# ethz-asl/object_keypoints

Measured on AMD Instinct MI355X. Metric: frames/sec keypoint inference (511x511 -> heatmaps+3D), higher is better.
Workload: dtype bf16; 1 GPU; BASELINE configs[2]: batch=64/GPU synthetic 511x511 frames, bf16 activations+weights, fp32 accumulate, CornerNet-Squeeze K=3 (valve) random-init procedural weights; fp32 NCHW frames -> stem -> hourglass+heads; peak-NMS -> depth lifting -> object grouping on injected bump scenes (SURVEY 8(d), 1-2 objects/frame); frames_per_gpu=64, global_batch=64, parallelism=frame-dp1, resident_frame_batches=4

## Files before the change

### object_keypoints_amd/csrc/okp_igemm_patch.hip

```cpp
#include <cstdio>
#include <cstdlib>
#include <cstring>
#include <type_traits>
#include <vector>

#include "okp_igemm_kernel.h"


namespace {

constexpr uint32_t kPatchKeys = 0x7ac788u;
template <int MT> __device__ __forceinline__ uint32_t patch_key(int col) {
  return MT == 16 ? (kPatchKeys >> (3 * (col >> 1))) & 7u : (uint32_t)(col >> 1) & 7u;
}

constexpr int kWStage = 256 * 128;
constexpr int kPitch = 18;
constexpr int kPatchBuf = 41 * 1024;
constexpr int kLdsPatch = 2 * kWStage;
constexpr int kLdsSteps = kLdsPatch + 2 * kPatchBuf;
constexpr int kLdsBias = kLdsSteps + 256 * (int)sizeof(OkpPatchStep);
#ifdef OKP_PATCH_STAMPS
constexpr int kStampBytes = 1024;
__device__ __forceinline__ uint64_t stamp() { uint64_t t; asm volatile("s_memtime %0" : "=s"(t)); return t; }
#else
constexpr int kStampBytes = 0;
#endif
constexpr int kGeoEntries = 328;
constexpr int kLdsGeo = kLdsBias + 1024;
constexpr int kLdsStamps = kLdsGeo + OKP_PATCH_MAX_GEOM * kGeoEntries * 4;
constexpr int kLdsTotal = kLdsStamps + kStampBytes;
static_assert(sizeof(OkpPatchStep) == 16, "step table entries are read as one 16-byte vector");
static_assert(256 * 512 <= kLdsSteps, "epilogue staging (256 px x 256 ch bf16) must not reach the step table");
static_assert(kLdsTotal <= 160 * 1024, "one workgroup's LDS is at most the CU's 160 KiB");

template <typename T, int MT = 16, bool RG = false>
__global__ __launch_bounds__(512) void okp_igemm_patch_kernel(const OkpPatchParams p) {
  static_assert(!RG || std::is_same<T, _Float16>::value, "the 16-bit storage guard is an fp16 instantiation");
  using x4_t = typename H16<T>::x4;
  using x8_t = typename H16<T>::x8;
  static_assert(MT == 16 || MT == 32, "MFMA tile");
  constexpr int TCO = 64 / MT, TPX = 128 / MT;
  constexpr int AREGS = MT * MT / 64;
  using acc_t = typename Mma<T, MT>::acc_t;
  __shared__ __attribute__((aligned(16))) char smem[kLdsTotal];
  char* const steps_lds = smem + kLdsSteps;
  char* const bias_lds = smem + kLdsBias;

  const int tid = threadIdx.x;
  const int lane = tid & 63;
  const int wave = __builtin_amdgcn_readfirstlane(tid >> 6);
  const int wco = wave >> 1, wpx = wave & 1;
  const int fr = lane & 15, fh = lane >> 4;

  const __amdgpu_buffer_rsrc_t rs_w = __builtin_amdgcn_make_buffer_rsrc(const_cast<void*>(p.weights), 0, (int)p.w_bytes, 0x00020000);
  const __amdgpu_buffer_rsrc_t rs_b = __builtin_amdgcn_make_buffer_rsrc(const_cast<float*>(p.bias), 0, p.n_co_tiles * 256 * 4, 0x00020000);
  const __amdgpu_buffer_rsrc_t rs_s0 = __builtin_amdgcn_make_buffer_rsrc(const_cast<void*>(p.src_data[0]), 0, (int)p.src_bytes[0], 0x00020000);
  const __amdgpu_buffer_rsrc_t rs_s1 = __builtin_amdgcn_make_buffer_rsrc(const_cast<void*>(p.src_data[1]), 0, (int)p.src_bytes[1], 0x00020000);

  if (tid < p.n_steps) reinterpret_cast<u32x4*>(steps_lds)[tid] = reinterpret_cast<const u32x4*>(p.steps)[tid];
  __syncthreads();

  const int r0 = tid >> 3;
  const int wc = (tid & 7) ^ ((r0 >> 1) & 7);

  for (int slot = blockIdx.x; slot < p.n_tiles; slot += gridDim.x) {
    const int xq = p.n_tiles >> 3, xr = p.n_tiles & 7, xcd = slot & 7;
    const int tile = (xcd < xr ? xcd * (xq + 1) : xr * (xq + 1) + (xcd - xr) * xq) + (slot >> 3);
    const int cls = p.n_classes == 4 ? (tile & 3) : 0;
    const int tile_c = p.n_classes == 4 ? (tile >> 2) : tile;
    const int t0 = cls * p.steps_per_class, t1 = t0 + p.steps_per_class;
    const int co_tile = tile_c % p.n_co_tiles;
    const int px_tile = tile_c / p.n_co_tiles;
    const int n = fastdiv(px_tile, p.div_tiles_frame);
    const int trem = px_tile - n * p.tiles_y * p.tiles_x;
    const int tyi = fastdiv(trem, p.div_tiles_x);
    const int y0 = tyi * 16, x0 = (trem - tyi * p.tiles_x) * 16;
    const int co0 = co_tile * 256;

    if (wave == 0)
      __builtin_amdgcn_raw_ptr_buffer_load_lds(rs_b, (lds_ptr_t)bias_lds, 16, (int)((uint32_t)(co0 + lane * 4) * 4u), 0, 0, 0);

    uint32_t wbase[4];
#pragma unroll
    for (int i = 0; i < 4; ++i) {
      const int co = co0 + r0 + i * 64;
      wbase[i] = (co < p.cout_pad) ? (uint32_t)co * 128u + (uint32_t)wc * 16u : kInvalidOff;
    }

    auto issue_w = [&](int t, int stage) {
      const uint32_t wslice = (uint32_t)t * (uint32_t)p.cout_pad * 128u;
      char* const wt = smem + stage * kWStage + wave * 1024;
#pragma unroll
      for (int i = 0; i < 4; ++i)
        __builtin_amdgcn_raw_ptr_buffer_load_lds(rs_w, (lds_ptr_t)(wt + i * 8192), 16, (int)(wbase[i] + wslice), 0, 0, 0);
    };
    auto patch_pixel = [&](const OkpPatchGeom& G, int idx) -> uint32_t {
      const int i = idx / kPitch, j = idx - i * kPitch;
      const int ys = G.conv_stride * y0 + G.oy + i * G.step, xs = G.conv_stride * x0 + G.ox + j * G.step;
      const bool ok = idx < G.npx && j < G.PW && ys >= 0 && ys < G.H && xs >= 0 && xs < G.W;
      return ok ? ((uint32_t)((n * G.H + ys) * G.W + xs) * (uint32_t)(G.pix_stride * 2)) | patch_key<MT>(j) : kInvalidOff;
    };
    auto issue_patch_tab = [&](int geom, uint32_t c0b, int k0, int k1, int buf) {
      const int npx = 18 * (int)((p.geom_ph >> (5 * geom)) & 31u);
      const __amdgpu_buffer_rsrc_t rs_x = ((p.geom_src >> geom) & 1) ? rs_s1 : rs_s0;
      const uint32_t* const tab = reinterpret_cast<const uint32_t*>(smem + kLdsGeo) + geom * kGeoEntries + (lane >> 3);
      for (int k = k0; k < k1; ++k) {
        const int blk = k * 8 + wave;
        if (blk * 8 >= npx) continue;
        const uint32_t e = tab[blk * 8];
        const uint32_t off = (e & kInvalidOff) ? kInvalidOff : (e & ~7u) + c0b + ((((uint32_t)lane & 7u) ^ (e & 7u)) << 4);
        __builtin_amdgcn_raw_ptr_buffer_load_lds(rs_x, (lds_ptr_t)(smem + kLdsPatch + buf * kPatchBuf + blk * 1024), 16, (int)off, 0, 0, 0);
      }
    };
    auto issue_patch = [&](int geom, uint32_t c0b, int k0, int k1, int buf) {
      const OkpPatchGeom& G = p.g[geom];
      const int PW = G.PW, npx = G.npx;
      const int H = G.H, W = G.W, ps2 = G.pix_stride * 2, step = G.step;
      const int yb = G.conv_stride * y0 + G.oy, xb = G.conv_stride * x0 + G.ox;
      const __amdgpu_buffer_rsrc_t rs_x = __builtin_amdgcn_make_buffer_rsrc(const_cast<void*>(G.data), 0, (int)G.bytes, 0x00020000);
      for (int k = k0; k < k1; ++k) {
        const int blk = k * 8 + wave;
        if (blk * 8 >= npx) continue;
        const int idx = blk * 8 + (lane >> 3);
        const int i = idx / kPitch, j = idx - i * kPitch;
        const int ch = (lane & 7) ^ (int)patch_key<MT>(j);
        const int ys = yb + i * step, xs = xb + j * step;
        const bool ok = idx < npx && j < PW && ys >= 0 && ys < H && xs >= 0 && xs < W;
        const uint32_t off = ok ? (uint32_t)((n * H + ys) * W + xs) * (uint32_t)ps2 + c0b + (uint32_t)ch * 16u : kInvalidOff;
        char* const dst = smem + kLdsPatch + buf * kPatchBuf + blk * 1024;
        __builtin_amdgcn_raw_ptr_buffer_load_lds(rs_x, (lds_ptr_t)dst, 16, (int)off, 0, 0, 0);
      }
    };

    acc_t acc[TCO][TPX];
#pragma unroll
    for (int i = 0; i < TCO; ++i)
#pragma unroll
      for (int j = 0; j < TPX; ++j)
#pragma unroll
        for (int e = 0; e < AREGS; ++e) acc[i][j][e] = 0.f;

    for (int g = 0; g < p.n_geom; ++g)
      if (tid < kGeoEntries) reinterpret_cast<uint32_t*>(smem + kLdsGeo)[g * kGeoEntries + tid] = patch_pixel(p.g[g], tid);
    {
      const u32x4 s0 = *reinterpret_cast<const u32x4*>(steps_lds + t0 * 16);
      const uint32_t w3 = (uint32_t)__builtin_amdgcn_readfirstlane((int)s0[3]);
      const int g0 = w3 & 0xff;
      issue_patch(g0, ((w3 >> 16) & 0xffu) * 128u, 0, (p.g[g0].npx + 63) >> 6, __builtin_amdgcn_readfirstlane((int)s0[2]) & 0xff);
    }
    issue_w(t0, t0 & 1);

    for (int t = t0; t < t1; ++t) {
      const u32x4 sv = *reinterpret_cast<const u32x4*>(steps_lds + t * 16);
      const uint32_t tap_bytes = (uint32_t)__builtin_amdgcn_readfirstlane((int)sv[0]);
      const uint32_t nx_c0b = (uint32_t)__builtin_amdgcn_readfirstlane((int)sv[1]);
      const uint32_t pk = (uint32_t)__builtin_amdgcn_readfirstlane((int)sv[2]);
      const int pbuf = pk & 0xff, nx_k0 = (pk >> 8) & 0xff, nx_k1 = (pk >> 16) & 0xff, nx_geom = pk >> 24;
      const uint32_t w3 = (uint32_t)__builtin_amdgcn_readfirstlane((int)sv[3]);
      const int dxo = (w3 >> 8) & 0xff;
      const bool more = t + 1 < t1;
#ifdef OKP_PATCH_ABL_NOPATCH
      const bool next_patch = false; (void)nx_k0; (void)nx_k1; (void)nx_geom; (void)nx_c0b;
#else
      const bool next_patch = nx_k1 > nx_k0 && (int)(w3 >> 24) + 1 < t1;
#endif

#ifdef OKP_PATCH_STAMPS
      uint64_t T0 = stamp();
      asm volatile("s_waitcnt vmcnt(0) lgkmcnt(0)" ::: "memory");
      uint64_t T1 = stamp();
      asm volatile("s_waitcnt lgkmcnt(0)" ::: "memory");
      __builtin_amdgcn_s_barrier();
      uint64_t T2 = stamp();
#else
      asm volatile("s_waitcnt vmcnt(0) lgkmcnt(0)" ::: "memory");
      __builtin_amdgcn_s_barrier();
#endif

      const char* const wt = smem + (t & 1) * kWStage;
      const char* const pbase = smem + kLdsPatch + pbuf * kPatchBuf;
      if constexpr (MT == 32) {
        const int r32 = lane & 31, h32 = lane >> 5;
        const char* const bb = pbase + tap_bytes + (uint32_t)(((wpx * 8 + (r32 >> 4)) * kPitch + (r32 & 15)) * 128);
        const uint32_t bsw = patch_key<32>((r32 & 15) + dxo);
        auto lda = [&](int sub, int i) { return *reinterpret_cast<const u32x4*>(wt + swz<128>((wco * TCO + i) * 32 + r32, 2 * sub + h32)); };
        auto ldb = [&](int sub, int j) { return *reinterpret_cast<const u32x4*>(bb + j * (2 * kPitch * 128) + ((((uint32_t)(2 * sub + h32)) ^ bsw) << 4)); };
        u32x4 fa[2][TCO], fb[2][TPX];
#pragma unroll
        for (int i = 0; i < TCO; ++i) fa[0][i] = lda(0, i);
#pragma unroll
        for (int j = 0; j < TPX; ++j) fb[0][j] = ldb(0, j);
        if (more) issue_w(t + 1, (t + 1) & 1);
#pragma unroll
        for (int sub = 0; sub < 4; ++sub) {
          __builtin_amdgcn_sched_barrier(0);
          if (sub + 1 < 4) {
#pragma unroll
            for (int i = 0; i < TCO; ++i) fa[(sub + 1) & 1][i] = lda(sub + 1, i);
#pragma unroll
            for (int j = 0; j < TPX; ++j) fb[(sub + 1) & 1][j] = ldb(sub + 1, j);
          }
          if (sub == 1 && next_patch) issue_patch_tab(nx_geom, nx_c0b, nx_k0, nx_k1, pbuf ^ 1);
          __builtin_amdgcn_sched_barrier(0);
#pragma unroll
          for (int i = 0; i < TCO; ++i)
#pragma unroll
            for (int j = 0; j < TPX; ++j) acc[i][j] = H16<T>::mfma32(fa[sub & 1][i], fb[sub & 1][j], acc[i][j]);
        }
      } else {
      const char* const bb = pbase + tap_bytes + (uint32_t)((wpx * TPX * kPitch + fr) * 128);
      const uint32_t bsw = patch_key<16>(fr + dxo);
      auto lda = [&](int kk, int i) {
        return *reinterpret_cast<const u32x4*>(wt + swz<128>((wco * TCO + i) * 16 + fr, 4 * kk + fh));
      };
      auto ldb = [&](int kk, int j) {
        return *reinterpret_cast<const u32x4*>(bb + j * (kPitch * 128) + ((((uint32_t)(4 * kk + fh)) ^ bsw) << 4));
      };
      auto mma8 = [&](const u32x4 (&a)[TCO], const u32x4 (&bq)[2], auto s) {
        constexpr int S = decltype(s)::value;
#pragma unroll
        for (int i = 0; i < TCO; ++i)
#pragma unroll
          for (int h = 0; h < 2; ++h)
            acc[i][2 * S + h] = H16<T>::mfma16(a[i], bq[h], acc[i][2 * S + h]);
      };
      using S0 = std::integral_constant<int, 0>; using S1 = std::integral_constant<int, 1>;
      using S2 = std::integral_constant<int, 2>; using S3 = std::integral_constant<int, 3>;
      u32x4 a0[TCO], a1[TCO], bq0[2], bq1[2];
#pragma unroll
      for (int i = 0; i < TCO; ++i) a0[i] = lda(0, i);
      bq0[0] = ldb(0, 0); bq0[1] = ldb(0, 1);
      bq1[0] = ldb(0, 2); bq1[1] = ldb(0, 3);
      if (more) issue_w(t + 1, (t + 1) & 1);
      __builtin_amdgcn_sched_barrier(0);
      mma8(a0, bq0, S0{});
      __builtin_amdgcn_sched_barrier(0);
#ifdef OKP_PATCH_STAMPS
      {
        uint64_t T3 = stamp();
        asm volatile("s_waitcnt lgkmcnt(0)" : "+s"(T0), "+s"(T1), "+s"(T2), "+s"(T3) :: "memory");
        if (slot == (int)blockIdx.x && lane == 0 && t - t0 < kStampBytes / 128)
          *reinterpret_cast<u32x4*>(smem + kLdsStamps + ((t - t0) * 8 + wave) * 16) = u32x4{(uint32_t)T0, (uint32_t)T1, (uint32_t)T2, (uint32_t)T3};
      }
      __builtin_amdgcn_sched_barrier(0);
#endif
      bq0[0] = ldb(0, 4); bq0[1] = ldb(0, 5); a1[0] = lda(1, 0); a1[1] = lda(1, 1);
      __builtin_amdgcn_sched_barrier(0);
      mma8(a0, bq1, S1{});
      __builtin_amdgcn_sched_barrier(0);
      bq1[0] = ldb(0, 6); bq1[1] = ldb(0, 7); a1[2] = lda(1, 2); a1[3] = lda(1, 3);
      __builtin_amdgcn_sched_barrier(0);
      mma8(a0, bq0, S2{});
      __builtin_amdgcn_sched_barrier(0);
      bq0[0] = ldb(1, 0); bq0[1] = ldb(1, 1);
      if (next_patch) issue_patch_tab(nx_geom, nx_c0b, nx_k0, nx_k1, pbuf ^ 1);
      __builtin_amdgcn_sched_barrier(0);
      mma8(a0, bq1, S3{});
      __builtin_amdgcn_sched_barrier(0);
      bq1[0] = ldb(1, 2); bq1[1] = ldb(1, 3);
      __builtin_amdgcn_sched_barrier(0);
      mma8(a1, bq0, S0{});
      __builtin_amdgcn_sched_barrier(0);
      bq0[0] = ldb(1, 4); bq0[1] = ldb(1, 5);
      __builtin_amdgcn_sched_barrier(0);
      mma8(a1, bq1, S1{});
      __builtin_amdgcn_sched_barrier(0);
      bq1[0] = ldb(1, 6); bq1[1] = ldb(1, 7);
      __builtin_amdgcn_sched_barrier(0);
      mma8(a1, bq0, S2{});
      mma8(a1, bq1, S3{});
          }
    }
#ifdef OKP_PATCH_STAMPS
    {
      uint64_t TE = stamp();
      asm volatile("s_waitcnt lgkmcnt(0)" : "+s"(TE) :: "memory");
      if (slot == (int)blockIdx.x && lane == 0 && t1 - t0 < kStampBytes / 128)
        *reinterpret_cast<u32x4*>(smem + kLdsStamps + ((t1 - t0) * 8 + wave) * 16) = u32x4{(uint32_t)TE, 0u, 0u, 0u};
    }
    __syncthreads();
    if (slot == (int)blockIdx.x && blockIdx.x < 16 && p.dbg)
      for (int i = tid; i < kStampBytes / 4; i += 512) p.dbg[blockIdx.x * (kStampBytes / 4) + i] = reinterpret_cast<const uint32_t*>(smem + kLdsStamps)[i];
#endif
    __syncthreads();

#pragma unroll
    for (int i = 0; i < TCO; ++i) {
#pragma unroll
      for (int g = 0; g < AREGS / 4; ++g) {
        const int co_l = (wco * TCO + i) * MT + (MT == 32 ? 8 * g + 4 * (lane >> 5) : 4 * fh);
        const f32x4 bv = *reinterpret_cast<const f32x4*>(bias_lds + co_l * 4);
#pragma unroll
        for (int j = 0; j < TPX; ++j) {
          const int prow = (wpx * TPX + j) * MT + (lane & (MT - 1));
          char* dst = smem + prow * 512 + ((((co_l * 2) >> 4) ^ (prow & 7)) << 4) + ((co_l * 2) & 15);
          x4_t o;
#pragma unroll
          for (int e = 0; e < 4; ++e) o[e] = (T)(acc[i][j][4 * g + e] + bv[e]);
          *reinterpret_cast<x4_t*>(dst) = o;
        }
      }
    }
    __syncthreads();
    constexpr int U = 256 * 32 / 512;
    constexpr int UH = 8;
    const bool relu = p.act == OKP_ACT_RELU;
    uint32_t range_h = 0u;
#pragma unroll 1
    for (int ub = 0; ub < U; ub += UH) {
      u32x4 rres[UH];
      uint32_t ooff[UH];
#pragma unroll
      for (int u = 0; u < UH; ++u) {
        const int it = tid + (ub + u) * 512;
        const int q = it & 31, prow = it >> 5;
        const int co = co0 + q * 8;
        const uint32_t opix = (uint32_t)((n * p.OH + (y0 + (prow >> 4)) * p.out_step + p.out_oy + (cls >> 1)) * p.OW + (x0 + (prow & 15)) * p.out_step + p.out_ox + (cls & 1));
        ooff[u] = co < p.cout ? opix : kInvalidOff;
      }
      if (p.res) {
#pragma unroll
        for (int u = 0; u < UH; ++u) {
          const int q = (tid + (ub + u) * 512) & 31;
          const int co = co0 + q * 8;
          const uint32_t opix = ooff[u] == kInvalidOff ? 0u : ooff[u];
          rres[u] = *reinterpret_cast<const u32x4*>(static_cast<const char*>(p.res) + ((size_t)opix * p.res_pix_stride + (co < p.cout ? co : 0)) * 2);
        }
      }
#pragma unroll
      for (int u = 0; u < UH; ++u) {
        const int it = tid + (ub + u) * 512;
        const int q = it & 31, prow = it >> 5;
        u32x4 w = *reinterpret_cast<const u32x4*>(smem + prow * 512 + ((q ^ (prow & 7)) << 4));
        if (ooff[u] == kInvalidOff) continue;
        char* op = static_cast<char*>(p.out) + ((size_t)ooff[u] * p.out_pix_stride + co0 + q * 8) * 2;
        if (!p.res) {
          if (relu) {
            typedef short s16x8 __attribute__((ext_vector_type(8)));
            const s16x8 z = {0, 0, 0, 0, 0, 0, 0, 0};
            w = __builtin_bit_cast(u32x4, __builtin_elementwise_max(__builtin_bit_cast(s16x8, w), z));
          }
          if constexpr (RG) range_h = okp_range_max_h8(range_h, w);
          *reinterpret_cast<u32x4*>(op) = w;
        } else {
          const x8_t s8 = __builtin_bit_cast(x8_t, w), r8 = __builtin_bit_cast(x8_t, rres[u]);
          x8_t o;
#pragma unroll
          for (int e = 0; e < 8; ++e) {
            float v = (float)s8[e] + (float)r8[e];
            if (relu) v = fmaxf(v, 0.f);
            o[e] = (T)v;
          }
          if constexpr (RG) range_h = okp_range_max_h8(range_h, __builtin_bit_cast(u32x4, o));
          *reinterpret_cast<x8_t*>(op) = o;
        }
      }
    }
    if constexpr (RG) okp_raise_range_flag(p.range_flag, okp_range_exceeded_h2(range_h));
    __syncthreads();
  }
}

}

bool okp_patch_supported(const okp_conv* plan, const OkpIgemmParams& p) {
  const bool x3 = plan->dtype == OKP_F32X3;
  if (!plan->patch_steps_dev || !(okp_is16(plan->dtype) || x3)) return false;
  if ((p.n_classes != 1 && p.n_classes != 4) || p.dw_w) return false;
  if (p.Ho % 16 || p.Wo % 16) return false;
  if (x3 && (p.out16 || p.res16 || p.out_sub2 || !p.out || plan->n_single_slices)) return false;
  for (int s = 0; s < plan->n_src; ++s) {
    if (p.src_pix_stride[s] < plan->cin[s]) return false;
    if ((p.src_pix_stride[s] * okp_esz(plan->dtype)) % 8) return false;
  }
  return true;
}

int okp_fill_patch_params(const okp_conv* plan, const OkpIgemmParams& q, OkpPatchParams& p) {
  std::memset(&p, 0, sizeof(p));
  for (int gi = 0; gi < plan->patch_n_geom; ++gi) {
    const int ss = plan->patch_src[gi];
    OkpPatchGeom& g = p.g[gi];
// ... 16 lines not shown
  p.weights = q.weights; p.w_bytes = q.w_bytes; p.cout_pad = q.cout_pad; p.cout = q.cout; p.bias = q.bias; p.oscale = q.oscale;
  p.steps = plan->patch_steps_dev; p.n_steps = plan->n_slices;
  p.n_classes = q.n_classes; p.steps_per_class = plan->n_slices / q.n_classes;
  p.OH = q.OH; p.OW = q.OW; p.out_step = q.out_step; p.out_oy = q.out_oy; p.out_ox = q.out_ox;
  p.N = q.N; p.H = q.Ho; p.W = q.Wo; p.tiles_y = q.Ho / 16; p.tiles_x = q.Wo / 16;
  p.div_tiles_frame = okp_fastdiv((uint32_t)(p.tiles_y * p.tiles_x)); p.div_tiles_x = okp_fastdiv((uint32_t)p.tiles_x);
  p.out = q.out; p.out_bytes = q.out_bytes; p.out_pix_stride = q.out_pix_stride;
  p.res = q.res; p.res_bytes = q.res_bytes; p.res_pix_stride = q.res_pix_stride; p.act = q.act;
  p.pairs = ((uint32_t)q.src_pairs & 3u) | (q.out_pairs ? 4u : 0u);
  p.range_flag = q.range_flag;
  p.n_co_tiles = q.cout_pad / 256;
  p.tiles_per_class = p.n_co_tiles * p.N * p.tiles_y * p.tiles_x;
  p.n_tiles = p.tiles_per_class * p.n_classes;
  return OKP_OK;
}

int okp_launch_igemm_patch(const okp_conv* plan, const OkpIgemmParams& q, hipStream_t stream) {
  if (!okp_patch_supported(plan, q)) { okp_set_error("okp_conv_forward: tile 13 (patch-resident kernel) does not apply to this plan / problem"); return OKP_EINVAL; }
  OkpPatchParams p;
  if (int e = okp_fill_patch_params(plan, q, p)) return e;
  if (plan->dtype == OKP_F32X3) return okp_launch_igemm_patch_x3(plan, p, stream);
#ifdef OKP_PATCH_STAMPS
  static uint32_t* dbg = nullptr;
  if (!dbg) (void)hipMalloc((void**)&dbg, 16 * kStampBytes);
  (void)hipMemsetAsync(dbg, 0, 16 * kStampBytes, stream);
  p.dbg = dbg;
#endif
  const dim3 grid((unsigned)(p.n_tiles < 256 ? p.n_tiles : 256)), block(512);
  if (q.mfma32) {
    if (plan->dtype == OKP_BF16) hipLaunchKernelGGL((okp_igemm_patch_kernel<__bf16, 32>), grid, block, 0, stream, p);
    else if (p.range_flag) hipLaunchKernelGGL((okp_igemm_patch_kernel<_Float16, 32, true>), grid, block, 0, stream, p);
    else hipLaunchKernelGGL((okp_igemm_patch_kernel<_Float16, 32>), grid, block, 0, stream, p);
  } else if (plan->dtype == OKP_BF16) hipLaunchKernelGGL((okp_igemm_patch_kernel<__bf16, 16>), grid, block, 0, stream, p);
  else if (p.range_flag) hipLaunchKernelGGL((okp_igemm_patch_kernel<_Float16, 16, true>), grid, block, 0, stream, p);
  else hipLaunchKernelGGL((okp_igemm_patch_kernel<_Float16, 16>), grid, block, 0, stream, p);
#ifdef OKP_PATCH_STAMPS
  if (getenv("OKP_PATCH_STAMPS_PRINT")) {
    (void)hipStreamSynchronize(stream);
    std::vector<uint32_t> h(16 * kStampBytes / 4);
    (void)hipMemcpy(h.data(), dbg, 16 * kStampBytes, hipMemcpyDeviceToHost);
    const int ns = std::min(p.steps_per_class, kStampBytes / 128 - 1);
    printf("patch stamps: %d K-steps per tile; clocks per step: wait for the LDS-DMA | barrier | until the first MFMA group was issued | rest of the body\n", p.steps_per_class);
    for (int wg = 0; wg < 16; wg += 5)
      for (int t = 0; t < ns; ++t) {
        printf("wg %2d step %2d:", wg, t);
        for (int w = 0; w < 8; w += 7) {
          const uint32_t* a = &h[(size_t)wg * (kStampBytes / 4) + (t * 8 + w) * 4];
          printf("   wave %d: %5u | %5u | %5u | %5u", w, a[1] - a[0], a[2] - a[1], a[3] - a[2], a[32] - a[3]);
        }
        printf("\n");
      }
    double sum[4] = {0, 0, 0, 0};
    int cnt = 0;
    for (int wg = 0; wg < 16; ++wg)
      for (int t = 1; t < ns; ++t)
        for (int w = 0; w < 8; ++w) {
          const uint32_t* a = &h[(size_t)wg * (kStampBytes / 4) + (t * 8 + w) * 4];
          sum[0] += a[1] - a[0]; sum[1] += a[2] - a[1]; sum[2] += a[3] - a[2]; sum[3] += a[32] - a[3]; ++cnt;
        }
    printf("mean over 16 workgroups, all waves, steps 1..: wait %.0f | barrier %.0f | first MFMAs %.0f | rest %.0f  = %.0f clocks per step\n",
           sum[0] / cnt, sum[1] / cnt, sum[2] / cnt, sum[3] / cnt, (sum[0] + sum[1] + sum[2] + sum[3]) / cnt);
  }
#endif
  return okp_check_hip(hipGetLastError(), "okp_igemm_patch launch");
}
```

Baseline: 12990 frames/s.

## Overlap patch kernel epilogue stores with next tile's prologue via register epilogue

Restructures the persistent patch-resident implicit-GEMM kernel so that for 16x16 MFMA tiles the epilogue writes directly from registers (weight rows permuted to match) instead of staging through LDS. The next tile's bias/weight/patch DMA is issued before the previous tile's stores drain, with a partial vmcnt wait that tolerates outstanding epilogue stores. The step table is loaded via LDS-DMA without a barrier. The aim is to hide the tile-boundary bubble (LDS staging, barriers, cold prologue). The cost is more complex wait-count logic and a risk of less coalesced global stores.

```diff
diff --git a/object_keypoints_amd/csrc/okp_igemm_patch.hip b/object_keypoints_amd/csrc/okp_igemm_patch.hip
--- a/object_keypoints_amd/csrc/okp_igemm_patch.hip
+++ b/object_keypoints_amd/csrc/okp_igemm_patch.hip
@@ -31,18 +31,25 @@
 constexpr int kLdsStamps = kLdsGeo + OKP_PATCH_MAX_GEOM * kGeoEntries * 4;
 constexpr int kLdsTotal = kLdsStamps + kStampBytes;
 static_assert(sizeof(OkpPatchStep) == 16, "step table entries are read as one 16-byte vector");
-static_assert(256 * 512 <= kLdsSteps, "epilogue staging (256 px x 256 ch bf16) must not reach the step table");
+static_assert(256 * 512 <= kLdsSteps, "MT == 32: epilogue staging (256 px x 256 ch bf16) must not reach the step table");
 static_assert(kLdsTotal <= 160 * 1024, "one workgroup's LDS is at most the CU's 160 KiB");
+
+struct PatchTile {
+  int cls, n, y0, x0, co0, t0, t1;
+};
 
 template <typename T, int MT = 16, bool RG = false>
 __global__ __launch_bounds__(512) void okp_igemm_patch_kernel(const OkpPatchParams p) {
   static_assert(!RG || std::is_same<T, _Float16>::value, "the 16-bit storage guard is an fp16 instantiation");
-  using x4_t = typename H16<T>::x4;
+  using x4_t [[maybe_unused]] = typename H16<T>::x4;
   using x8_t = typename H16<T>::x8;
   static_assert(MT == 16 || MT == 32, "MFMA tile");
   constexpr int TCO = 64 / MT, TPX = 128 / MT;
   constexpr int AREGS = MT * MT / 64;
+  constexpr bool REG_EPI = MT == 16;
+  constexpr int kEpiStores = 2 * TPX;
   using acc_t = typename Mma<T, MT>::acc_t;
+  using True = std::integral_constant<bool, true>; using False = std::integral_constant<bool, false>;
   __shared__ __attribute__((aligned(16))) char smem[kLdsTotal];
   char* const steps_lds = smem + kLdsSteps;
   char* const bias_lds = smem + kLdsBias;
@@ -58,157 +65,175 @@
   const __amdgpu_buffer_rsrc_t rs_s0 = __builtin_amdgcn_make_buffer_rsrc(const_cast<void*>(p.src_data[0]), 0, (int)p.src_bytes[0], 0x00020000);
   const __amdgpu_buffer_rsrc_t rs_s1 = __builtin_amdgcn_make_buffer_rsrc(const_cast<void*>(p.src_data[1]), 0, (int)p.src_bytes[1], 0x00020000);
 
-  if (tid < p.n_steps) reinterpret_cast<u32x4*>(steps_lds)[tid] = reinterpret_cast<const u32x4*>(p.steps)[tid];
-  __syncthreads();
+  if constexpr (REG_EPI) {
+    const __amdgpu_buffer_rsrc_t rs_t = __builtin_amdgcn_make_buffer_rsrc(const_cast<OkpPatchStep*>(p.steps), 0, p.n_steps * 16, 0x00020000);
+    if (wave < 4) __builtin_amdgcn_raw_ptr_buffer_load_lds(rs_t, (lds_ptr_t)(steps_lds + wave * 1024), 16, tid * 16, 0, 0, 0);
+  } else {
+    if (tid < p.n_steps) reinterpret_cast<u32x4*>(steps_lds)[tid] = reinterpret_cast<const u32x4*>(p.steps)[tid];
+    __syncthreads();
+  }
 
   const int r0 = tid >> 3;
   const int wc = (tid & 7) ^ ((r0 >> 1) & 7);
-
-  for (int slot = blockIdx.x; slot < p.n_tiles; slot += gridDim.x) {
+  const int wrow = REG_EPI ? 32 * (r0 >> 5) + 8 * ((r0 >> 2) & 3) + 4 * ((r0 >> 4) & 1) + (r0 & 3) : r0;
+
+  auto tile_of = [&](int slot) -> PatchTile {
     const int xq = p.n_tiles >> 3, xr = p.n_tiles & 7, xcd = slot & 7;
     const int tile = (xcd < xr ? xcd * (xq + 1) : xr * (xq + 1) + (xcd - xr) * xq) + (slot >> 3);
-    const int cls = p.n_classes == 4 ? (tile & 3) : 0;
+    PatchTile q;
+    q.cls = p.n_classes == 4 ? (tile & 3) : 0;
     const int tile_c = p.n_classes == 4 ? (tile >> 2) : tile;
-    const int t0 = cls * p.steps_per_class, t1 = t0 + p.steps_per_class;
+    q.t0 = q.cls * p.steps_per_class; q.t1 = q.t0 + p.steps_per_class;
     const int co_tile = tile_c % p.n_co_tiles;
     const int px_tile = tile_c / p.n_co_tiles;
-    const int n = fastdiv(px_tile, p.div_tiles_frame);
-    const int trem = px_tile - n * p.tiles_y * p.tiles_x;
+    q.n = fastdiv(px_tile, p.div_tiles_frame);
+    const int trem = px_tile - q.n * p.tiles_y * p.tiles_x;
     const int tyi = fastdiv(trem, p.div_tiles_x);
-    const int y0 = tyi * 16, x0 = (trem - tyi * p.tiles_x) * 16;
-    const int co0 = co_tile * 256;
-
+    q.y0 = tyi * 16; q.x0 = (trem - tyi * p.tiles_x) * 16;
+    q.co0 = co_tile * 256;
+    return q;
+  };
+
+  uint32_t wbase[4];
+  auto issue_w = [&](int t, int stage) {
+    const uint32_t wslice = (uint32_t)t * (uint32_t)p.cout_pad * 128u;
+    char* const wt = smem + stage * kWStage + wave * 1024;
+#pragma unroll
+    for (int i = 0; i < 4; ++i)
+      __builtin_amdgcn_raw_ptr_buffer_load_lds(rs_w, (lds_ptr_t)(wt + i * 8192), 16, (int)(wbase[i] + wslice), 0, 0, 0);
+  };
+  auto patch_pixel = [&](const PatchTile& q, const OkpPatchGeom& G, int idx) -> uint32_t {
+    const int i = idx / kPitch, j = idx - i * kPitch;
+    const int ys = G.conv_stride * q.y0 + G.oy + i * G.step, xs = G.conv_stride * q.x0 + G.ox + j * G.step;
+    const bool ok = idx < G.npx && j < G.PW && ys >= 0 && ys < G.H && xs >= 0 && xs < G.W;
+    return ok ? ((uint32_t)((q.n * G.H + ys) * G.W + xs) * (uint32_t)(G.pix_stride * 2)) | patch_key<MT>(j) : kInvalidOff;
+  };
+  auto issue_patch_tab = [&](int geom, uint32_t c0b, int k0, int k1, int buf) {
+    const int npx = 18 * (int)((p.geom_ph >> (5 * geom)) & 31u);
+    const __amdgpu_buffer_rsrc_t rs_x = ((p.geom_src >> geom) & 1) ? rs_s1 : rs_s0;
+    const uint32_t* const tab = reinterpret_cast<const uint32_t*>(smem + kLdsGeo) + geom * kGeoEntries + (lane >> 3);
+    for (int k = k0; k < k1; ++k) {
+      const int blk = k * 8 + wave;
+      if (blk * 8 >= npx) continue;
+      const uint32_t e = tab[blk * 8];
+      const uint32_t off = (e & kInvalidOff) ? kInvalidOff : (e & ~7u) + c0b + ((((uint32_t)lane & 7u) ^ (e & 7u)) << 4);
+      __builtin_amdgcn_raw_ptr_buffer_load_lds(rs_x, (lds_ptr_t)(smem + kLdsPatch + buf * kPatchBuf + blk * 1024), 16, (int)off, 0, 0, 0);
+    }
+  };
+  auto issue_patch = [&](const PatchTile& q, int geom, uint32_t c0b, int k0, int k1, int buf) {
+    const OkpPatchGeom& G = p.g[geom];
+    const int PW = G.PW, npx = G.npx;
+    const int H = G.H, W = G.W, ps2 = G.pix_stride * 2, step = G.step;
+    const int yb = G.conv_stride * q.y0 + G.oy, xb = G.conv_stride * q.x0 + G.ox;
+    const __amdgpu_buffer_rsrc_t rs_x = __builtin_amdgcn_make_buffer_rsrc(const_cast<void*>(G.data), 0, (int)G.bytes, 0x00020000);
+    for (int k = k0; k < k1; ++k) {
+      const int blk = k * 8 + wave;
+      if (blk * 8 >= npx) continue;
+      const int idx = blk * 8 + (lane >> 3);
+      const int i = idx / kPitch, j = idx - i * kPitch;
+      const int ch = (lane & 7) ^ (int)patch_key<MT>(j);
+      const int ys = yb + i * step, xs = xb + j * step;
+      const bool ok = idx < npx && j < PW && ys >= 0 && ys < H && xs >= 0 && xs < W;
+      const uint32_t off = ok ? (uint32_t)((q.n * H + ys) * W + xs) * (uint32_t)ps2 + c0b + (uint32_t)ch * 16u : kInvalidOff;
+      char* const dst = smem + kLdsPatch + buf * kPatchBuf + blk * 1024;
+      __builtin_amdgcn_raw_ptr_buffer_load_lds(rs_x, (lds_ptr_t)dst, 16, (int)off, 0, 0, 0);
+    }
+  };
+  auto tile_begin = [&](const PatchTile& q, auto first_tag) -> u32x4 {
+    constexpr bool FIRST = decltype(first_tag)::value;
     if (wave == 0)
-      __builtin_amdgcn_raw_ptr_buffer_load_lds(rs_b, (lds_ptr_t)bias_lds, 16, (int)((uint32_t)(co0 + lane * 4) * 4u), 0, 0, 0);
-
-    uint32_t wbase[4];
+      __builtin_amdgcn_raw_ptr_buffer_load_lds(rs_b, (lds_ptr_t)bias_lds, 16, (int)((uint32_t)(q.co0 + lane * 4) * 4u), 0, 0, 0);
 #pragma unroll
     for (int i = 0; i < 4; ++i) {
-      const int co = co0 + r0 + i * 64;
+      const int co = q.co0 + wrow + i * 64;
       wbase[i] = (co < p.cout_pad) ? (uint32_t)co * 128u + (uint32_t)wc * 16u : kInvalidOff;
     }
-
-    auto issue_w = [&](int t, int stage) {
-      const uint32_t wslice = (uint32_t)t * (uint32_t)p.cout_pad * 128u;
-      char* const wt = smem + stage * kWStage + wave * 1024;
-#pragma unroll
-      for (int i = 0; i < 4; ++i)
-        __builtin_amdgcn_raw_ptr_buffer_load_lds(rs_w, (lds_ptr_t)(wt + i * 8192), 16, (int)(wbase[i] + wslice), 0, 0, 0);
+    for (int g = 0; g < p.n_geom; ++g)
+      if (tid < kGeoEntries) reinterpret_cast<uint32_t*>(smem + kLdsGeo)[g * kGeoEntries + tid] = patch_pixel(q, p.g[g], tid);
+    u32x4 s0;
+    if constexpr (FIRST) s0 = *reinterpret_cast<const u32x4*>(p.steps + q.t0);
+    else s0 = *reinterpret_cast<const u32x4*>(steps_lds + q.t0 * 16);
+#pragma unroll
+    for (int e = 0; e < 4; ++e) s0[e] = (uint32_t)__builtin_amdgcn_readfirstlane((int)s0[e]);
+    const uint32_t w3 = s0[3];
+    const int g0 = w3 & 0xff;
+    issue_patch(q, g0, ((w3 >> 16) & 0xffu) * 128u, 0, (p.g[g0].npx + 63) >> 6, (int)(s0[2] & 0xff));
+    issue_w(q.t0, q.t0 & 1);
+    return s0;
+  };
+
+  acc_t acc[TCO][TPX];
+  int round = 0;
+#ifdef OKP_PATCH_STAMPS
+  uint32_t TB0 = 0, TB1 = 0;
+#endif
+
+  auto kstep = [&](const int t, const int t0, const int t1, const u32x4 sv, auto peel_tag) {
+    constexpr bool PEEL = decltype(peel_tag)::value;
+    const uint32_t tap_bytes = (uint32_t)__builtin_amdgcn_readfirstlane((int)sv[0]);
+    const uint32_t nx_c0b = (uint32_t)__builtin_amdgcn_readfirstlane((int)sv[1]);
+    const uint32_t pk = (uint32_t)__builtin_amdgcn_readfirstlane((int)sv[2]);
+    const int pbuf = pk & 0xff, nx_k0 = (pk >> 8) & 0xff, nx_k1 = (pk >> 16) & 0xff, nx_geom = pk >> 24;
+    const uint32_t w3 = (uint32_t)__builtin_amdgcn_readfirstlane((int)sv[3]);
+    const int dxo = (w3 >> 8) & 0xff;
+    const bool more = t + 1 < t1;
+#ifdef OKP_PATCH_ABL_NOPATCH
+    const bool next_patch = false; (void)nx_k0; (void)nx_k1; (void)nx_geom; (void)nx_c0b;
+#else
+    const bool next_patch = nx_k1 > nx_k0 && (int)(w3 >> 24) + 1 < t1;
+#endif
+
+    auto wait_dma = [&]() {
+      if constexpr (PEEL && REG_EPI) {
+        if (round > 0) asm volatile("s_waitcnt vmcnt(%0) lgkmcnt(0)" ::"n"(kEpiStores) : "memory");
+        else asm volatile("s_waitcnt vmcnt(0) lgkmcnt(0)" ::: "memory");
+      } else {
+        asm volatile("s_waitcnt vmcnt(0) lgkmcnt(0)" ::: "memory");
+      }
     };
-    auto patch_pixel = [&](const OkpPatchGeom& G, int idx) -> uint32_t {
-      const int i = idx / kPitch, j = idx - i * kPitch;
-      const int ys = G.conv_stride * y0 + G.oy + i * G.step, xs = G.conv_stride * x0 + G.ox + j * G.step;
-      const bool ok = idx < G.npx && j < G.PW && ys >= 0 && ys < G.H && xs >= 0 && xs < G.W;
-      return ok ? ((uint32_t)((n * G.H + ys) * G.W + xs) * (uint32_t)(G.pix_stride * 2)) | patch_key<MT>(j) : kInvalidOff;
-    };
-    auto issue_patch_tab = [&](int geom, uint32_t c0b, int k0, int k1, int buf) {
-      const int npx = 18 * (int)((p.geom_ph >> (5 * geom)) & 31u);
-      const __amdgpu_buffer_rsrc_t rs_x = ((p.geom_src >> geom) & 1) ? rs_s1 : rs_s0;
-      const uint32_t* const tab = reinterpret_cast<const uint32_t*>(smem + kLdsGeo) + geom * kGeoEntries + (lane >> 3);
-      for (int k = k0; k < k1; ++k) {
-        const int blk = k * 8 + wave;
-        if (blk * 8 >= npx) continue;
-        const uint32_t e = tab[blk * 8];
-        const uint32_t off = (e & kInvalidOff) ? kInvalidOff : (e & ~7u) + c0b + ((((uint32_t)lane & 7u) ^ (e & 7u)) << 4);
-        __builtin_amdgcn_raw_ptr_buffer_load_lds(rs_x, (lds_ptr_t)(smem + kLdsPatch + buf * kPatchBuf + blk * 1024), 16, (int)off, 0, 0, 0);
-      }
-    };
-    auto issue_patch = [&](int geom, uint32_t c0b, int k0, int k1, int buf) {
-      const OkpPatchGeom& G = p.g[geom];
-      const int PW = G.PW, npx = G.npx;
-      const int H = G.H, W = G.W, ps2 = G.pix_stride * 2, step = G.step;
-      const int yb = G.conv_stride * y0 + G.oy, xb = G.conv_stride * x0 + G.ox;
-      const __amdgpu_buffer_rsrc_t rs_x = __builtin_amdgcn_make_buffer_rsrc(const_cast<void*>(G.data), 0, (int)G.bytes, 0x00020000);
-      for (int k = k0; k < k1; ++k) {
-        const int blk = k * 8 + wave;
-        if (blk * 8 >= npx) continue;
-        const int idx = blk * 8 + (lane >> 3);
-        const int i = idx / kPitch, j = idx - i * kPitch;
-        const int ch = (lane & 7) ^ (int)patch_key<MT>(j);
-        const int ys = yb + i * step, xs = xb + j * step;
-        const bool ok = idx < npx && j < PW && ys >= 0 && ys < H && xs >= 0 && xs < W;
-        const uint32_t off = ok ? (uint32_t)((n * H + ys) * W + xs) * (uint32_t)ps2 + c0b + (uint32_t)ch * 16u : kInvalidOff;
-        char* const dst = smem + kLdsPatch + buf * kPatchBuf + blk * 1024;
-        __builtin_amdgcn_raw_ptr_buffer_load_lds(rs_x, (lds_ptr_t)dst, 16, (int)off, 0, 0, 0);
-      }
-    };
-
-    acc_t acc[TCO][TPX];
-#pragma unroll
-    for (int i = 0; i < TCO; ++i)
-#pragma unroll
-      for (int j = 0; j < TPX; ++j)
-#pragma unroll
-        for (int e = 0; e < AREGS; ++e) acc[i][j][e] = 0.f;
-
-    for (int g = 0; g < p.n_geom; ++g)
-      if (tid < kGeoEntries) reinterpret_cast<uint32_t*>(smem + kLdsGeo)[g * kGeoEntries + tid] = patch_pixel(p.g[g], tid);
-    {
-      const u32x4 s0 = *reinterpret_cast<const u32x4*>(steps_lds + t0 * 16);
-      const uint32_t w3 = (uint32_t)__builtin_amdgcn_readfirstlane((int)s0[3]);
-      const int g0 = w3 & 0xff;
-      issue_patch(g0, ((w3 >> 16) & 0xffu) * 128u, 0, (p.g[g0].npx + 63) >> 6, __builtin_amdgcn_readfirstlane((int)s0[2]) & 0xff);
-    }
-    issue_w(t0, t0 & 1);
-
-    for (int t = t0; t < t1; ++t) {
-      const u32x4 sv = *reinterpret_cast<const u32x4*>(steps_lds + t * 16);
-      const uint32_t tap_bytes = (uint32_t)__builtin_amdgcn_readfirstlane((int)sv[0]);
-      const uint32_t nx_c0b = (uint32_t)__builtin_amdgcn_readfirstlane((int)sv[1]);
-      const uint32_t pk = (uint32_t)__builtin_amdgcn_readfirstlane((int)sv[2]);
-      const int pbuf = pk & 0xff, nx_k0 = (pk >> 8) & 0xff, nx_k1 = (pk >> 16) & 0xff, nx_geom = pk >> 24;
-      const uint32_t w3 = (uint32_t)__builtin_amdgcn_readfirstlane((int)sv[3]);
-      const int dxo = (w3 >> 8) & 0xff;
-      const bool more = t + 1 < t1;
-#ifdef OKP_PATCH_ABL_NOPATCH
-      const bool next_patch = false; (void)nx_k0; (void)nx_k1; (void)nx_geom; (void)nx_c0b;
+#ifdef OKP_PATCH_STAMPS
+    uint64_t T0 = stamp();
+    wait_dma();
+    uint64_t T1 = stamp();
+    asm volatile("s_waitcnt lgkmcnt(0)" ::: "memory");
+    __builtin_amdgcn_s_barrier();
+    uint64_t T2 = stamp();
 #else
-      const bool next_patch = nx_k1 > nx_k0 && (int)(w3 >> 24) + 1 < t1;
-#endif
-
-#ifdef OKP_PATCH_STAMPS
-      uint64_t T0 = stamp();
-      asm volatile("s_waitcnt vmcnt(0) lgkmcnt(0)" ::: "memory");
-      uint64_t T1 = stamp();
-      asm volatile("s_waitcnt lgkmcnt(0)" ::: "memory");
-      __builtin_amdgcn_s_barrier();
-      uint64_t T2 = stamp();
-#else
-      asm volatile("s_waitcnt vmcnt(0) lgkmcnt(0)" ::: "memory");
-      __builtin_amdgcn_s_barrier();
-#endif
-
-      const char* const wt = smem + (t & 1) * kWStage;
-      const char* const pbase = smem + kLdsPatch + pbuf * kPatchBuf;
-      if constexpr (MT == 32) {
-        const int r32 = lane & 31, h32 = lane >> 5;
-        const char* const bb = pbase + tap_bytes + (uint32_t)(((wpx * 8 + (r32 >> 4)) * kPitch + (r32 & 15)) * 128);
-        const uint32_t bsw = patch_key<32>((r32 & 15) + dxo);
-        auto lda = [&](int sub, int i) { return *reinterpret_cast<const u32x4*>(wt + swz<128>((wco * TCO + i) * 32 + r32, 2 * sub + h32)); };
-        auto ldb = [&](int sub, int j) { return *reinterpret_cast<const u32x4*>(bb + j * (2 * kPitch * 128) + ((((uint32_t)(2 * sub + h32)) ^ bsw) << 4)); };
-        u32x4 fa[2][TCO], fb[2][TPX];
-#pragma unroll
-        for (int i = 0; i < TCO; ++i) fa[0][i] = lda(0, i);
-#pragma unroll
-        for (int j = 0; j < TPX; ++j) fb[0][j] = ldb(0, j);
-        if (more) issue_w(t + 1, (t + 1) & 1);
-#pragma unroll
-        for (int sub = 0; sub < 4; ++sub) {
-          __builtin_amdgcn_sched_barrier(0);
-          if (sub + 1 < 4) {
-#pragma unroll
-            for (int i = 0; i < TCO; ++i) fa[(sub + 1) & 1][i] = lda(sub + 1, i);
-#pragma unroll
-            for (int j = 0; j < TPX; ++j) fb[(sub + 1) & 1][j] = ldb(sub + 1, j);
-          }
-          if (sub == 1 && next_patch) issue_patch_tab(nx_geom, nx_c0b, nx_k0, nx_k1, pbuf ^ 1);
-          __builtin_amdgcn_sched_barrier(0);
-#pragma unroll
-          for (int i = 0; i < TCO; ++i)
-#pragma unroll
-            for (int j = 0; j < TPX; ++j) acc[i][j] = H16<T>::mfma32(fa[sub & 1][i], fb[sub & 1][j], acc[i][j]);
-        }
-      } else {
+    wait_dma();
+    __builtin_amdgcn_s_barrier();
+#endif
+
+    const char* const wt = smem + (t & 1) * kWStage;
+    const char* const pbase = smem + kLdsPatch + pbuf * kPatchBuf;
+    if constexpr (MT == 32) {
+      const int r32 = lane & 31, h32 = lane >> 5;
+      const char* const bb = pbase + tap_bytes + (uint32_t)(((wpx * 8 + (r32 >> 4)) * kPitch + (r32 & 15)) * 128);
+      const uint32_t bsw = patch_key<32>((r32 & 15) + dxo);
+      auto lda = [&](int sub, int i) { return *reinterpret_cast<const u32x4*>(wt + swz<128>((wco * TCO + i) * 32 + r32, 2 * sub + h32)); };
+      auto ldb = [&](int sub, int j) { return *reinterpret_cast<const u32x4*>(bb + j * (2 * kPitch * 128) + ((((uint32_t)(2 * sub + h32)) ^ bsw) << 4)); };
+      u32x4 fa[2][TCO], fb[2][TPX];
+#pragma unroll
+      for (int i = 0; i < TCO; ++i) fa[0][i] = lda(0, i);
+#pragma unroll
+      for (int j = 0; j < TPX; ++j) fb[0][j] = ldb(0, j);
+      if (more) issue_w(t + 1, (t + 1) & 1);
+#pragma unroll
+      for (int sub = 0; sub < 4; ++sub) {
+        __builtin_amdgcn_sched_barrier(0);
+        if (sub + 1 < 4) {
+#pragma unroll
+          for (int i = 0; i < TCO; ++i) fa[(sub + 1) & 1][i] = lda(sub + 1, i);
+#pragma unroll
+          for (int j = 0; j < TPX; ++j) fb[(sub + 1) & 1][j] = ldb(sub + 1, j);
+        }
+        if (sub == 1 && next_patch) issue_patch_tab(nx_geom, nx_c0b, nx_k0, nx_k1, pbuf ^ 1);
+        __builtin_amdgcn_sched_barrier(0);
+#pragma unroll
+        for (int i = 0; i < TCO; ++i)
+#pragma unroll
+          for (int j = 0; j < TPX; ++j) acc[i][j] = H16<T>::mfma32(fa[sub & 1][i], fb[sub & 1][j], acc[i][j]);
+      }
+    } else {
       const char* const bb = pbase + tap_bytes + (uint32_t)((wpx * TPX * kPitch + fr) * 128);
       const uint32_t bsw = patch_key<16>(fr + dxo);
       auto lda = [&](int kk, int i) {
@@ -240,8 +265,10 @@
       {
         uint64_t T3 = stamp();
         asm volatile("s_waitcnt lgkmcnt(0)" : "+s"(T0), "+s"(T1), "+s"(T2), "+s"(T3) :: "memory");
-        if (slot == (int)blockIdx.x && lane == 0 && t - t0 < kStampBytes / 128)
+        if (round == 0 && lane == 0 && t - t0 < kStampBytes / 128)
           *reinterpret_cast<u32x4*>(smem + kLdsStamps + ((t - t0) * 8 + wave) * 16) = u32x4{(uint32_t)T0, (uint32_t)T1, (uint32_t)T2, (uint32_t)T3};
+        if (PEEL && round == 1 && lane == 0 && blockIdx.x < 16 && p.dbg)
+          *reinterpret_cast<u32x4*>(p.dbg + 16 * (kStampBytes / 4) + (blockIdx.x * 8 + wave) * 4) = u32x4{TB0, TB1, (uint32_t)T3, 1u};
       }
       __builtin_amdgcn_sched_barrier(0);
 #endif
@@ -270,95 +297,215 @@
       __builtin_amdgcn_sched_barrier(0);
       mma8(a1, bq0, S2{});
       mma8(a1, bq1, S3{});
+    }
+  };
+  auto zero_acc = [&]() {
+#pragma unroll
+    for (int i = 0; i < TCO; ++i)
+#pragma unroll
+      for (int j = 0; j < TPX; ++j)
+#pragma unroll
+        for (int e = 0; e < AREGS; ++e) acc[i][j][e] = 0.f;
+  };
+#ifdef OKP_PATCH_STAMPS
+  auto stamp_loop_end = [&](const PatchTile& q) {
+    uint64_t TE = stamp();
+    asm volatile("s_waitcnt lgkmcnt(0)" : "+s"(TE) :: "memory");
+    TB0 = (uint32_t)TE;
+    if (round == 0 && lane == 0 && q.t1 - q.t0 < kStampBytes / 128)
+      *reinterpret_cast<u32x4*>(smem + kLdsStamps + ((q.t1 - q.t0) * 8 + wave) * 16) = u32x4{(uint32_t)TE, 0u, 0u, 0u};
+    __syncthreads();
+    if (round == 0 && blockIdx.x < 16 && p.dbg)
+      for (int i = tid; i < kStampBytes / 4; i += 512) p.dbg[blockIdx.x * (kStampBytes / 4) + i] = reinterpret_cast<const uint32_t*>(smem + kLdsStamps)[i];
+  };
+#endif
+
+  if constexpr (REG_EPI) {
+    const __amdgpu_buffer_rsrc_t rs_o = __builtin_amdgcn_make_buffer_rsrc(p.out, 0, (int)p.out_bytes, 0x00020000);
+    const __amdgpu_buffer_rsrc_t rs_r = __builtin_amdgcn_make_buffer_rsrc(const_cast<void*>(p.res), 0, (int)p.res_bytes, 0x00020000);
+    const bool relu = p.act == OKP_ACT_RELU;
+    PatchTile tl = tile_of(blockIdx.x);
+    u32x4 s0 = tile_begin(tl, True{});
+    for (int slot = blockIdx.x;;) {
+      zero_acc();
+      kstep(tl.t0, tl.t0, tl.t1, s0, True{});
+      for (int t = tl.t0 + 1; t < tl.t1; ++t) kstep(t, tl.t0, tl.t1, *reinterpret_cast<const u32x4*>(steps_lds + t * 16), False{});
+#ifdef OKP_PATCH_STAMPS
+      stamp_loop_end(tl);
+#endif
+      f32x4 bv[2][2];
+#pragma unroll
+      for (int h = 0; h < 2; ++h)
+#pragma unroll
+        for (int q = 0; q < 2; ++q) bv[h][q] = *reinterpret_cast<const f32x4*>(bias_lds + (64 * wco + 32 * h + 8 * fh + 4 * q) * 4);
+      asm volatile("s_waitcnt lgkmcnt(0)" ::: "memory");
+      __builtin_amdgcn_s_barrier();
+      const PatchTile ep = tl;
+      const int nslot = slot + (int)gridDim.x;
+      const bool has_next = nslot < p.n_tiles;
+      if (has_next) {
+        tl = tile_of(nslot);
+        s0 = tile_begin(tl, False{});
+      }
+
+      {
+        const uint32_t ops2 = (uint32_t)p.out_pix_stride * 2u, rps2 = (uint32_t)p.res_pix_stride * 2u;
+        const uint32_t opix = (uint32_t)((ep.n * p.OH + (ep.y0 + 8 * wpx) * p.out_step + p.out_oy + (ep.cls >> 1)) * p.OW + (ep.x0 + fr) * p.out_step + p.out_ox + (ep.cls & 1));
+        const uint32_t orow = (uint32_t)(p.out_step * p.OW);
+        uint32_t ooff[2], roff[2], okm[2];
+#pragma unroll
+        for (int h = 0; h < 2; ++h) {
+          const int co = ep.co0 + 64 * wco + 32 * h + 8 * fh;
+          const bool ok = co < p.cout;
+          ooff[h] = ok ? opix * ops2 + (uint32_t)co * 2u : kInvalidOff;
+          roff[h] = ok ? opix * rps2 + (uint32_t)co * 2u : kInvalidOff;
+          okm[h] = ok ? 0xffffffffu : 0u;
+        }
+        uint32_t range_h = 0u;
+        auto packed = [&](int j, int h) -> x8_t {
+          x8_t o;
+#pragma unroll
+          for (int e = 0; e < 8; ++e) o[e] = (T)(acc[2 * h + (e >> 2)][j][e & 3] + bv[h][e >> 2][e & 3]);
+          return o;
+        };
+        if (!p.res) {
+#pragma unroll
+          for (int j = 0; j < TPX; ++j)
+#pragma unroll
+            for (int h = 0; h < 2; ++h) {
+              u32x4 w = __builtin_bit_cast(u32x4, packed(j, h));
+              if (relu) {
+                typedef short s16x8 __attribute__((ext_vector_type(8)));
+                const s16x8 z = {0, 0, 0, 0, 0, 0, 0, 0};
+                w = __builtin_bit_cast(u32x4, __builtin_elementwise_max(__builtin_bit_cast(s16x8, w), z));
+              }
+              if constexpr (RG) range_h = okp_range_max_h8(range_h, u32x4{w[0] & okm[h], w[1] & okm[h], w[2] & okm[h], w[3] & okm[h]});
+              __builtin_amdgcn_raw_buffer_store_b128(w, rs_o, (int)(ooff[h] + (uint32_t)j * orow * ops2), 0, 0);
+            }
+        } else {
+          constexpr int UJ = 4;
+#pragma unroll
+          for (int jb = 0; jb < TPX; jb += UJ) {
+            u32x4 rres[UJ][2];
+#pragma unroll
+            for (int j = 0; j < UJ; ++j)
+#pragma unroll
+              for (int h = 0; h < 2; ++h)
+                rres[j][h] = __builtin_amdgcn_raw_buffer_load_b128(rs_r, (int)(roff[h] + (uint32_t)(jb + j) * orow * rps2), 0, 0);
+#pragma unroll
+            for (int j = 0; j < UJ; ++j)
+#pragma unroll
+              for (int h = 0; h < 2; ++h) {
+                const x8_t s8 = packed(jb + j, h), r8 = __builtin_bit_cast(x8_t, rres[j][h]);
+                x8_t o;
+#pragma unroll
+                for (int e = 0; e < 8; ++e) {
+                  float v = (float)s8[e] + (float)r8[e];
+                  if (relu) v = fmaxf(v, 0.f);
+                  o[e] = (T)v;
+                }
+                const u32x4 w = __builtin_bit_cast(u32x4, o);
+                if constexpr (RG) range_h = okp_range_max_h8(range_h, u32x4{w[0] & okm[h], w[1] & okm[h], w[2] & okm[h], w[3] & okm[h]});
+                __builtin_amdgcn_raw_buffer_store_b128(w, rs_o, (int)(ooff[h] + (uint32_t)(jb + j) * orow * ops2), 0, 0);
+              }
           }
+        }
+        if constexpr (RG) okp_raise_range_flag(p.range_flag, okp_range_exceeded_h2(range_h));
+      }
+#ifdef OKP_PATCH_STAMPS
+      { uint64_t TS = stamp(); asm volatile("s_waitcnt lgkmcnt(0)" : "+s"(TS) :: "memory"); TB1 = (uint32_t)TS; }
+#endif
+      if (!has_next) break;
+      slot = nslot;
+      ++round;
     }
-#ifdef OKP_PATCH_STAMPS
-    {
-      uint64_t TE = stamp();
-      asm volatile("s_waitcnt lgkmcnt(0)" : "+s"(TE) :: "memory");
-      if (slot == (int)blockIdx.x && lane == 0 && t1 - t0 < kStampBytes / 128)
-        *reinterpret_cast<u32x4*>(smem + kLdsStamps + ((t1 - t0) * 8 + wave) * 16) = u32x4{(uint32_t)TE, 0u, 0u, 0u};
+  } else {
+    for (int slot = blockIdx.x; slot < p.n_tiles; slot += gridDim.x, ++round) {
+      const PatchTile tl = tile_of(slot);
+      const int n = tl.n, y0 = tl.y0, x0 = tl.x0, co0 = tl.co0, cls = tl.cls;
+      (void)tile_begin(tl, False{});
+      zero_acc();
+      for (int t = tl.t0; t < tl.t1; ++t) kstep(t, tl.t0, tl.t1, *reinterpret_cast<const u32x4*>(steps_lds + t * 16), False{});
+#ifdef OKP_PATCH_STAMPS
+      stamp_loop_end(tl);
+#endif
+      __syncthreads();
+
+#pragma unroll
+      for (int i = 0; i < TCO; ++i) {
+#pragma unroll
+        for (int g = 0; g < AREGS / 4; ++g) {
+          const int co_l = (wco * TCO + i) * MT + (MT == 32 ? 8 * g + 4 * (lane >> 5) : 4 * fh);
+          const f32x4 bv = *reinterpret_cast<const f32x4*>(bias_lds + co_l * 4);
+#pragma unroll
+          for (int j = 0; j < TPX; ++j) {
+            const int prow = (wpx * TPX + j) * MT + (lane & (MT - 1));
+            char* dst = smem + prow * 512 + ((((co_l * 2) >> 4) ^ (prow & 7)) << 4) + ((co_l * 2) & 15);
+            x4_t o;
+#pragma unroll
+            for (int e = 0; e < 4; ++e) o[e] = (T)(acc[i][j][4 * g + e] + bv[e]);
+            *reinterpret_cast<x4_t*>(dst) = o;
+          }
+        }
+      }
+      __syncthreads();
+      constexpr int U = 256 * 32 / 512;
+      constexpr int UH = 8;
+      const bool relu = p.act == OKP_ACT_RELU;
+      uint32_t range_h = 0u;
+#pragma unroll 1
+      for (int ub = 0; ub < U; ub += UH) {
+        u32x4 rres[UH];
+        uint32_t ooff[UH];
+#pragma unroll
+        for (int u = 0; u < UH; ++u) {
+          const int it = tid + (ub + u) * 512;
+          const int q = it & 31, prow = it >> 5;
+          const int co = co0 + q * 8;
+          const uint32_t opix = (uint32_t)((n * p.OH + (y0 + (prow >> 4)) * p.out_step + p.out_oy + (cls >> 1)) * p.OW + (x0 + (prow & 15)) * p.out_step + p.out_ox + (cls & 1));
+          ooff[u] = co < p.cout ? opix : kInvalidOff;
+        }
+        if (p.res) {
+#pragma unroll
+          for (int u = 0; u < UH; ++u) {
+            const int q = (tid + (ub + u) * 512) & 31;
+            const int co = co0 + q * 8;
+            const uint32_t opix = ooff[u] == kInvalidOff ? 0u : ooff[u];
+            rres[u] = *reinterpret_cast<const u32x4*>(static_cast<const char*>(p.res) + ((size_t)opix * p.res_pix_stride + (co < p.cout ? co : 0)) * 2);
+          }
+        }
+#pragma unroll
+        for (int u = 0; u < UH; ++u) {
+          const int it = tid + (ub + u) * 512;
+          const int q = it & 31, prow = it >> 5;
+          u32x4 w = *reinterpret_cast<const u32x4*>(smem + prow * 512 + ((q ^ (prow & 7)) << 4));
+          if (ooff[u] == kInvalidOff) continue;
+          char* op = static_cast<char*>(p.out) + ((size_t)ooff[u] * p.out_pix_stride + co0 + q * 8) * 2;
+          if (!p.res) {
+            if (relu) {
+              typedef short s16x8 __attribute__((ext_vector_type(8)));
+              const s16x8 z = {0, 0, 0, 0, 0, 0, 0, 0};
+              w = __builtin_bit_cast(u32x4, __builtin_elementwise_max(__builtin_bit_cast(s16x8, w), z));
+            }
+            if constexpr (RG) range_h = okp_range_max_h8(range_h, w);
+            *reinterpret_cast<u32x4*>(op) = w;
+          } else {
+            const x8_t s8 = __builtin_bit_cast(x8_t, w), r8 = __builtin_bit_cast(x8_t, rres[u]);
+            x8_t o;
+#pragma unroll
+            for (int e = 0; e < 8; ++e) {
+              float v = (float)s8[e] + (float)r8[e];
+              if (relu) v = fmaxf(v, 0.f);
+              o[e] = (T)v;
+            }
+            if constexpr (RG) range_h = okp_range_max_h8(range_h, __builtin_bit_cast(u32x4, o));
+            *reinterpret_cast<x8_t*>(op) = o;
+          }
+        }
+      }
+      if constexpr (RG) okp_raise_range_flag(p.range_flag, okp_range_exceeded_h2(range_h));
+      __syncthreads();
     }
-    __syncthreads();
-    if (slot == (int)blockIdx.x && blockIdx.x < 16 && p.dbg)
-      for (int i = tid; i < kStampBytes / 4; i += 512) p.dbg[blockIdx.x * (kStampBytes / 4) + i] = reinterpret_cast<const uint32_t*>(smem + kLdsStamps)[i];
-#endif
-    __syncthreads();
-
-#pragma unroll
-    for (int i = 0; i < TCO; ++i) {
-#pragma unroll
-      for (int g = 0; g < AREGS / 4; ++g) {
-        const int co_l = (wco * TCO + i) * MT + (MT == 32 ? 8 * g + 4 * (lane >> 5) : 4 * fh);
-        const f32x4 bv = *reinterpret_cast<const f32x4*>(bias_lds + co_l * 4);
-#pragma unroll
-        for (int j = 0; j < TPX; ++j) {
-          const int prow = (wpx * TPX + j) * MT + (lane & (MT - 1));
-          char* dst = smem + prow * 512 + ((((co_l * 2) >> 4) ^ (prow & 7)) << 4) + ((co_l * 2) & 15);
-          x4_t o;
-#pragma unroll
-          for (int e = 0; e < 4; ++e) o[e] = (T)(acc[i][j][4 * g + e] + bv[e]);
-          *reinterpret_cast<x4_t*>(dst) = o;
-        }
-      }
-    }
-    __syncthreads();
-    constexpr int U = 256 * 32 / 512;
-    constexpr int UH = 8;
-    const bool relu = p.act == OKP_ACT_RELU;
-    uint32_t range_h = 0u;
-#pragma unroll 1
-    for (int ub = 0; ub < U; ub += UH) {
-      u32x4 rres[UH];
-      uint32_t ooff[UH];
-#pragma unroll
-      for (int u = 0; u < UH; ++u) {
-        const int it = tid + (ub + u) * 512;
-        const int q = it & 31, prow = it >> 5;
-        const int co = co0 + q * 8;
-        const uint32_t opix = (uint32_t)((n * p.OH + (y0 + (prow >> 4)) * p.out_step + p.out_oy + (cls >> 1)) * p.OW + (x0 + (prow & 15)) * p.out_step + p.out_ox + (cls & 1));
-        ooff[u] = co < p.cout ? opix : kInvalidOff;
-      }
-      if (p.res) {
-#pragma unroll
-        for (int u = 0; u < UH; ++u) {
-          const int q = (tid + (ub + u) * 512) & 31;
-          const int co = co0 + q * 8;
-          const uint32_t opix = ooff[u] == kInvalidOff ? 0u : ooff[u];
-          rres[u] = *reinterpret_cast<const u32x4*>(static_cast<const char*>(p.res) + ((size_t)opix * p.res_pix_stride + (co < p.cout ? co : 0)) * 2);
-        }
-      }
-#pragma unroll
-      for (int u = 0; u < UH; ++u) {
-        const int it = tid + (ub + u) * 512;
-        const int q = it & 31, prow = it >> 5;
-        u32x4 w = *reinterpret_cast<const u32x4*>(smem + prow * 512 + ((q ^ (prow & 7)) << 4));
-        if (ooff[u] == kInvalidOff) continue;
-        char* op = static_cast<char*>(p.out) + ((size_t)ooff[u] * p.out_pix_stride + co0 + q * 8) * 2;
-        if (!p.res) {
-          if (relu) {
-            typedef short s16x8 __attribute__((ext_vector_type(8)));
-            const s16x8 z = {0, 0, 0, 0, 0, 0, 0, 0};
-            w = __builtin_bit_cast(u32x4, __builtin_elementwise_max(__builtin_bit_cast(s16x8, w), z));
-          }
-          if constexpr (RG) range_h = okp_range_max_h8(range_h, w);
-          *reinterpret_cast<u32x4*>(op) = w;
-        } else {
-          const x8_t s8 = __builtin_bit_cast(x8_t, w), r8 = __builtin_bit_cast(x8_t, rres[u]);
-          x8_t o;
-#pragma unroll
-          for (int e = 0; e < 8; ++e) {
-            float v = (float)s8[e] + (float)r8[e];
-            if (relu) v = fmaxf(v, 0.f);
-            o[e] = (T)v;
-          }
-          if constexpr (RG) range_h = okp_range_max_h8(range_h, __builtin_bit_cast(u32x4, o));
-          *reinterpret_cast<x8_t*>(op) = o;
-        }
-      }
-    }
-    if constexpr (RG) okp_raise_range_flag(p.range_flag, okp_range_exceeded_h2(range_h));
-    __syncthreads();
   }
 }
 
@@ -421,8 +568,9 @@
   if (plan->dtype == OKP_F32X3) return okp_launch_igemm_patch_x3(plan, p, stream);
 #ifdef OKP_PATCH_STAMPS
   static uint32_t* dbg = nullptr;
-  if (!dbg) (void)hipMalloc((void**)&dbg, 16 * kStampBytes);
-  (void)hipMemsetAsync(dbg, 0, 16 * kStampBytes, stream);
+  constexpr int kDbgBytes = 16 * kStampBytes + 16 * 8 * 16;
+  if (!dbg) (void)hipMalloc((void**)&dbg, kDbgBytes);
+  (void)hipMemsetAsync(dbg, 0, kDbgBytes, stream);
   p.dbg = dbg;
 #endif
   const dim3 grid((unsigned)(p.n_tiles < 256 ? p.n_tiles : 256)), block(512);
@@ -436,8 +584,8 @@
 #ifdef OKP_PATCH_STAMPS
   if (getenv("OKP_PATCH_STAMPS_PRINT")) {
     (void)hipStreamSynchronize(stream);
-    std::vector<uint32_t> h(16 * kStampBytes / 4);
-    (void)hipMemcpy(h.data(), dbg, 16 * kStampBytes, hipMemcpyDeviceToHost);
+    std::vector<uint32_t> h(kDbgBytes / 4);
+    (void)hipMemcpy(h.data(), dbg, kDbgBytes, hipMemcpyDeviceToHost);
     const int ns = std::min(p.steps_per_class, kStampBytes / 128 - 1);
     printf("patch stamps: %d K-steps per tile; clocks per step: wait for the LDS-DMA | barrier | until the first MFMA group was issued | rest of the body\n", p.steps_per_class);
     for (int wg = 0; wg < 16; wg += 5)
@@ -459,6 +607,13 @@
         }
     printf("mean over 16 workgroups, all waves, steps 1..: wait %.0f | barrier %.0f | first MFMAs %.0f | rest %.0f  = %.0f clocks per step\n",
            sum[0] / cnt, sum[1] / cnt, sum[2] / cnt, sum[3] / cnt, (sum[0] + sum[1] + sum[2] + sum[3]) / cnt);
+    double bs[2] = {0, 0};
+    int bc = 0;
+    for (int i = 0; i < 16 * 8; ++i) {
+      const uint32_t* a = &h[(size_t)16 * (kStampBytes / 4) + i * 4];
+      if (a[3]) { bs[0] += a[1] - a[0]; bs[1] += a[2] - a[1]; ++bc; }
+    }
+    if (bc) printf("tile boundary, first -> second tile, mean over %d waves: K loop's end -> last store issued %.0f | -> first MFMA group of the next tile %.0f clocks\n", bc, bs[0] / bc, bs[1] / bc);
   }
 #endif
   return okp_check_hip(hipGetLastError(), "okp_igemm_patch launch");
```

New measurement: 12810 frames/s. 1.4% lower.
